# hyllios/CGAT

Measured on AMD Instinct MI355X. Metric: edges/sec through one CGAT attention layer (fwd+bwd), 1M-edge batch, higher is better.
Workload: dtype f32 storage / f16x3c (24-bit operands: exact h + l + t split, 3 fp16 + 3 six-bit matrix passes where built, six bf16 passes elsewhere; fp32 accumulate); 1 GPU; one GATConvNodes layer (H_Net update) fwd+bwd, 4167 crystals x 20 atoms x 12 nbrs per rank: N=83340, E=1000080, C=Ce=128, H=3, scalar attention; edges_per_rank=1000080, parallelism=dp1 (graphs sharded, gradient all-reduce)

## Files before the change

### cgat_amd/_lib.py

```python
import ctypes as C
import os

import torch

_HERE = os.path.dirname(os.path.abspath(__file__))
LIB_PATH = os.path.join(_HERE, "libcgat_hip.so")

MAX_FC = 8
MAX_HYPER = 8
ABI_VERSION = 3

ACT_NONE, ACT_TANH, ACT_LEAKY, ACT_RELU = 0, 1, 2, 3

c_float_p = C.POINTER(C.c_float)
c_i32_p = C.POINTER(C.c_int32)
c_i64_p = C.POINTER(C.c_int64)
vp = C.c_void_p


class Plan(C.Structure):
    _fields_ = [("N", C.c_int32), ("E", C.c_int32), ("dst_rowptr", vp), ("dst_perm", vp), ("dst_sorted", vp),
                ("src_sorted", vp), ("src_rowptr", vp), ("src_pos", vp)]


# ... 106 lines not shown
    "cgat_nodes_attention_bit_form": (C.c_int32, [C.POINTER(Plan), C.POINTER(AttnParams)]),
    "cgat_nodes_attention_infer_workspace_bytes": (C.c_size_t, [C.POINTER(Plan), C.POINTER(AttnParams)]),
    "cgat_nodes_attention_infer": (C.c_int, [C.POINTER(Plan), C.POINTER(AttnParams), vp, vp, vp, vp, C.c_size_t, vp]),
    "cgat_nodes_attention_infer_indexed_ok": (C.c_int32, [C.POINTER(Plan), C.POINTER(AttnParams), C.c_int32]),
    "cgat_nodes_attention_infer_indexed_workspace_bytes": (C.c_size_t, [C.POINTER(Plan), C.POINTER(AttnParams), C.c_int32]),
    "cgat_nodes_attention_infer_indexed": (C.c_int, [C.POINTER(Plan), C.POINTER(AttnParams), vp, vp, C.c_int32, vp, vp, vp,
                                                     C.c_size_t, vp]),
    "cgat_nodes_attention_train_indexed_ok": (C.c_int32, [C.POINTER(Plan), C.POINTER(AttnParams), C.c_int32]),
    "cgat_nodes_attention_indexed_saved_floats": (C.c_size_t, [C.c_int32, C.c_int32, C.c_int32, C.c_int32]),
    "cgat_nodes_attention_forward_indexed_workspace_bytes": (C.c_size_t, [C.POINTER(Plan), C.POINTER(AttnParams), C.c_int32]),
    "cgat_nodes_attention_forward_indexed": (C.c_int, [C.POINTER(Plan), C.POINTER(AttnParams), vp, vp, C.c_int32, vp, vp, vp,
                                                       vp, C.c_size_t, vp]),
    "cgat_nodes_attention_backward_indexed_workspace_bytes": (C.c_size_t, [C.POINTER(Plan), C.POINTER(AttnParams), C.c_int32]),
    "cgat_nodes_attention_backward_indexed": (C.c_int, [C.POINTER(Plan), C.POINTER(AttnParams), vp, vp, C.c_int32, vp, vp, vp,
                                                        vp, vp, vp, vp, vp, C.POINTER(AttnGrads), vp, C.c_size_t, vp]),
    "cgat_indexed_class_pieces": (C.c_int32, [C.c_int32, C.c_int32]),
    "cgat_indexed_class_plan_workspace_bytes": (C.c_size_t, [C.c_int32, C.c_int32]),
    "cgat_indexed_class_plan": (C.c_int, [C.POINTER(Plan), vp, C.c_int32, vp, vp, vp, vp, C.c_size_t, vp]),
    "cgat_debug_nodes_attention_signs_indexed_workspace_bytes": (C.c_size_t, [C.POINTER(Plan), C.POINTER(AttnParams),
                                                                              C.c_int32]),
    "cgat_debug_nodes_attention_signs_indexed": (C.c_int, [C.POINTER(Plan), C.POINTER(AttnParams), vp, vp, C.c_int32, vp, vp,
                                                           vp, C.c_size_t, vp]),
    "cgat_debug_nodes_attention_route": (C.c_uint32, [C.POINTER(Plan), C.POINTER(AttnParams), C.c_int32]),
    "cgat_debug_edge_z_form": (C.c_int, [C.c_int32] * 6 + [C.c_int64] + [C.c_int32] * 5 + [C.POINTER(EdgeZForm)]),
    "cgat_debug_edge_bwd_form": (C.c_int, [C.c_int32] * 11 + [C.POINTER(EdgeBwdForm)]),
    "cgat_debug_nodes_attention_signs": (C.c_int, [C.POINTER(Plan), C.POINTER(AttnParams), vp, vp, vp]),
    "cgat_debug_edge_ge_rebuilt_workspace_bytes": (C.c_size_t, [C.c_int32, C.c_int32, C.c_int32]),
    "cgat_debug_edge_ge_rebuilt": (C.c_int, [vp, vp, vp, vp, vp, vp, vp, C.c_int32, C.c_int32, C.c_int32, vp, vp,
                                             C.c_size_t, vp]),
    "cgat_debug_edge_gw_force_six": (C.c_int32, [C.c_int32]),
    "cgat_debug_edge_gw_rebuilt_workspace_bytes": (C.c_size_t, [C.c_int32, C.c_int32, C.c_int32]),
    "cgat_debug_edge_gw_rebuilt": (C.c_int, [vp, vp, vp, vp, vp, vp, vp, vp, C.c_int32, C.c_int32, C.c_int32, C.c_int32,
                                             vp, C.POINTER(C.c_int32), vp, C.c_size_t, vp]),
    "cgat_hnet_saved_floats": (C.c_size_t, [C.c_int32, C.POINTER(HnetParams)]),
    "cgat_hnet_forward_workspace_bytes": (C.c_size_t, [C.c_int32, C.POINTER(HnetParams)]),
    "cgat_hnet_backward_workspace_bytes": (C.c_size_t, [C.c_int32, C.POINTER(HnetParams)]),
    "cgat_hnet_forward": (C.c_int, [C.c_int32, C.POINTER(HnetParams), vp, vp, vp, vp, vp, C.c_size_t, vp]),
    "cgat_hnet_backward": (C.c_int, [C.c_int32, C.POINTER(HnetParams), vp, vp, vp, vp, vp, vp, C.POINTER(HnetGrads),
                                     vp, C.c_size_t, vp]),
    "cgat_hnet_backward_side_workspace_bytes": (C.c_size_t, [C.c_int32, C.POINTER(HnetParams)]),
    "cgat_hnet_backward_overlapped": (C.c_int, [C.c_int32, C.POINTER(HnetParams), vp, vp, vp, vp, vp, vp,
                                                C.POINTER(HnetGrads), vp, C.c_size_t, vp, vp, C.c_size_t, vp]),
    "cgat_debug_hnet_route": (C.c_uint32, [C.c_int32, C.POINTER(HnetParams), C.c_int32, C.c_int32]),
    "cgat_linear_backward_workspace_bytes": (C.c_size_t, [C.c_int32, C.c_int32, C.c_int32]),
    "cgat_linear_forward_workspace_bytes": (C.c_size_t, [C.c_int32, C.c_int32, C.c_int32]),
    "cgat_linear_forward": (C.c_int, [vp, C.c_int64, vp, C.c_int64, vp, vp, C.c_int64, C.c_int32, C.c_int32,
                                      C.c_int32, C.c_int32, vp, vp, C.c_size_t, vp]),
    "cgat_linear_backward": (C.c_int, [vp, C.c_int64, vp, C.c_int64, vp, C.c_int64, vp, C.c_int64, vp, vp, C.c_int64,
                                       C.c_int32, vp, C.c_int64, vp, C.c_int32, C.c_int32, C.c_int32, C.c_int32, vp,
                                       C.c_size_t, vp]),
    "cgat_segment_softmax_forward": (C.c_int, [vp, vp, vp, C.c_int32, C.c_int32, C.c_float, vp, vp]),
    "cgat_segment_softmax_backward": (C.c_int, [vp, vp, vp, vp, C.c_int32, C.c_int32, vp, vp, vp]),
    "cgat_segment_sum": (C.c_int, [vp, C.c_int64, vp, vp, C.c_int32, C.c_int32, vp, C.c_int64, vp]),
    "cgat_segment_attention_pool_forward": (C.c_int, [vp, C.c_int32, vp, vp, C.c_int64, vp, vp, C.c_int32, C.c_int32, C.c_float,
                                                      vp, vp, vp, vp, vp]),
    "cgat_segment_attention_pool_backward": (C.c_int, [vp, C.c_int32, vp, vp, C.c_int64, vp, vp, C.c_int32, C.c_int32, vp, vp, vp,
                                                       vp, vp, vp, vp, C.c_int64, vp, vp]),
    "cgat_segment_attention_pool_dropout_forward": (C.c_int, [vp, C.c_int32, vp, vp, vp, C.c_int64, vp, vp, C.c_int32,
                                                              C.c_int32, C.c_float, vp, vp, vp, vp, vp]),
    "cgat_segment_attention_pool_dropout_backward": (C.c_int, [vp, C.c_int32, vp, vp, vp, C.c_int64, vp, vp, C.c_int32,
                                                               C.c_int32, vp, vp, vp, vp, vp, vp, vp, C.c_int64, vp]),
    "cgat_edge_head_combine_forward": (C.c_int, [vp, C.c_int32, vp, vp, vp, C.c_int64, C.c_int32, C.c_int32, vp, vp]),
    "cgat_edge_head_combine_backward": (C.c_int, [vp, C.c_int32, vp, vp, vp, vp, C.c_int64, C.c_int32, C.c_int32, vp, vp,
                                                  vp]),
    "cgat_mlp_chain_workspace_bytes": (C.c_size_t, [C.c_int32]),
    "cgat_mlp_chain": (C.c_int, [C.POINTER(ChainDesc), vp, C.c_size_t, vp]),
    "cgat_rowprog_run": (C.c_int, [C.POINTER(RowProg), vp, vp]),
# ... 108 lines not shown
```

### cgat_amd/csrc/edgebwd.hip

```cpp
#include <string.h>
#include "../../include/cgat_hip.h"
#include "common.h"
#include "kernels.h"
#include "mfma_bf16.h"

__device__ __forceinline__ float rc_d(unsigned m, int bit) {
  const unsigned s = (unsigned)((int)(m << (31 - bit)) >> 31);
  return __uint_as_float((s & 0x3F800000u) | (~s & 0x3C23D70Au));
}
__device__ __forceinline__ bf16x8 bits8_bf16(unsigned m) {
  uint4 w;
#define GE_BITPAIR(i_) ((((unsigned)((int)(m << (31 - 2 * (i_))) >> 31)) & 0x3F80u) |                     \
                        (((unsigned)((int)(m << (30 - 2 * (i_))) >> 31)) & 0x3F800000u))
  w.x = GE_BITPAIR(0); w.y = GE_BITPAIR(1); w.z = GE_BITPAIR(2); w.w = GE_BITPAIR(3);
#undef GE_BITPAIR
  return __builtin_bit_cast(bf16x8, w);
}
template <int PASSES, bool RC = false, bool BP = false>
__global__ __launch_bounds__(512, 2) void edge_ge_kernel(const float* __restrict__ gZ, long ldg, long gzb,
                                                         const uint4* __restrict__ Wq, int ncb,
                                                         float* __restrict__ out, long ldo,
                                                         const int* __restrict__ scatter, int E, int accumulate,
                                                         const float* __restrict__ bias,
                                                         const float* __restrict__ amax, const EdgeRC rc, HeadBatch hb) {
// ... 985 lines not shown
}

int edge_gw_launch(const EdgeGwParams& p, hipStream_t stream) {
  if (p.E <= 0) {
    GemmParams z = gemm_params(p.W2, 128, 0, nullptr, 1, nullptr, 1, p.out, p.ldo);
    return gemm_launch(z, nullptr, 0, stream);
  }
  const EdgeGwForm f = edge_gw_form(p);
  CGAT_TRY(edge_gw_check(p, f));
  CGAT_TRY(prepare_T_bf16_rows_launch(p.e, p.lde, p.perm, p.E, p.ws, cdiv(p.E, 128), stream, f.passes == 2 ? p.emax : nullptr));
  if (f.bitplane || f.te_only) {
    {
      CGAT_PROF("edge_gw", stream);
      edge_gw_go(f, p, true, stream);
      CGAT_LAUNCH_CHECK();
    }
    hipLaunchKernelGGL(edge_gw_bit_reduce_kernel, dim3(p.W2 * 4), dim3(256), 0, stream, p.ws + f.slab, f.SM, p.ws + f.slabA, f.SA,
                       p.ws + f.csl, p.rc->wA, p.rc->H, p.rc->HHd, p.W2, f.te_only ? nullptr : p.out, p.ldo, p.te ? *p.te : GwTe{});
    CGAT_LAUNCH_CHECK();
    if (p.te) {
      hipLaunchKernelGGL(gw_te_add_kernel, dim3(cdiv(p.rc->HHd, 256)), dim3(256), 0, stream, p.te->part, p.rc->HHd, p.te->out);
      CGAT_LAUNCH_CHECK();
    }
    if (!f.te_only) return CGAT_OK;
  }
  {
    CGAT_PROF(p.perm ? "edge_gw" : "rows_gw", stream);
    edge_gw_go(f, p, false, stream);
    CGAT_LAUNCH_CHECK();
  }
  return splitk_reduce_launch(p.ws + f.slab, f.S, p.W2, 128, p.out, p.ldo, stream);
}

#define GJ_NODES 4
__global__ __launch_bounds__(256) void edge_gj_kernel(const EdgeRC rc, const int* __restrict__ src_rowptr,
                                                      const int* __restrict__ src_pos, int N, int W2,
                                                      float* __restrict__ Gj, long ldo, float* __restrict__ gjmax) {
  float gmax = 0.f;
  const int per_xcd = gridDim.x / 8;
  const int blk = (blockIdx.x & 7) * per_xcd + (blockIdx.x >> 3);
  const int n0 = blk * GJ_NODES, n1 = min(N, n0 + GJ_NODES);
  for (int q = threadIdx.x; 4 * q < W2; q += 256) {
    const int col = 4 * q;
    const bool isA = col < rc.HHd;
    const int cc = isA ? col : col - rc.HHd, h = cc / rc.Hd;
    const int word = col >> 5, bit = col & 31;
    const float* coef = (isA ? rc.ga : rc.alpha) + h;
    for (int n = n0; n < n1; ++n) {
      const int r0 = src_rowptr[n], r1 = src_rowptr[n + 1];
      float4 acc = make_float4(0.f, 0.f, 0.f, 0.f);
      for (int rb = r0; rb < r1; rb += 4) {
        long t[4];
        float k[4];
        unsigned m[4];
        float4 v[4];
#pragma unroll
        for (int u = 0; u < 4; ++u) t[u] = src_pos[rb + u < r1 ? rb + u : r1 - 1];
#pragma unroll
        for (int u = 0; u < 4; ++u) {
          k[u] = rb + u < r1 ? coef[t[u] * rc.H] : 0.f;
          m[u] = rc.mask[t[u] * rc.nw + word];
          v[u] = *reinterpret_cast<const float4*>(isA ? rc.wA + cc : rc.gS + (long)rc.dst[t[u]] * rc.HHd + cc);
        }
#pragma unroll
        for (int u = 0; u < 4; ++u) {
          const unsigned mb = m[u] >> bit;
          acc.x += (k[u] * v[u].x) * rc_d(mb, 0); acc.y += (k[u] * v[u].y) * rc_d(mb, 1);
          acc.z += (k[u] * v[u].z) * rc_d(mb, 2); acc.w += (k[u] * v[u].w) * rc_d(mb, 3);
        }
      }
      *reinterpret_cast<float4*>(Gj + (long)n * ldo + col) = acc;
      gmax = fmaxf(fmaxf(gmax, fmaxf(fabsf(acc.x), fabsf(acc.y))), fmaxf(fabsf(acc.z), fabsf(acc.w)));
    }
  }
  if (gjmax) block_absmax_commit(gmax, gjmax);
}
int edge_gj_launch(const EdgeRC& rc, const int* src_rowptr, const int* src_pos, int N, int W2, float* Gj, long ldo,
                   hipStream_t stream, float* gjmax) {
  if (N <= 0) return CGAT_OK;
  CGAT_CHECK_ARG(W2 % 4 == 0 && (ldo % 4) == 0 && (((uintptr_t)Gj) & 15) == 0,
                 "edge_gj: W2 = %d must be a multiple of 4 with a 16-byte aligned output", W2);
  CGAT_PROF("edge_gj", stream);
  hipLaunchKernelGGL(edge_gj_kernel, dim3(cdiv(cdiv(N, GJ_NODES), 8) * 8), dim3(256), 0, stream, rc, src_rowptr, src_pos,
                     N, W2, Gj, ldo, gjmax);
  CGAT_LAUNCH_CHECK();
  return CGAT_OK;
}

extern "C" int cgat_debug_edge_bwd_form(int32_t product, int32_t launch, int32_t rows, int32_t W2, int32_t H, int32_t Hd,
                                        int32_t rebuilt, int32_t maxima, int32_t perm, int32_t force_six, int32_t te,
                                        cgat_edge_bwd_form* out) {
  CGAT_CHECK_ARG(out && (product == 0 || product == 1) && launch >= 0 && launch <= (product == 0 ? 3 : 0) && rows >= 0 &&
                 W2 > 0 && W2 % 128 == 0 && H > 0 && Hd > 0, "debug_edge_bwd_form: bad arguments");
  alignas(16) static float present_f;
  static int present_i;
  const EdgeRC rc = edge_rc_shape_only(H, Hd, W2);
  memset(out, 0, sizeof(*out));
  if (product == 1) {
    const EdgeGwParams p = edge_gw_shape(rows, W2, rebuilt ? &rc : nullptr, maxima != 0, perm != 0, force_six != 0, te != 0);
    const EdgeGwForm f = edge_gw_form(p);
    CGAT_TRY(edge_gw_check(p, f));
    out->passes = f.passes; out->rc = f.rc; out->bitplane = f.bitplane; out->grid_x = f.grid_x;
    out->bit_shape = f.bit_shape; out->te_only = f.te_only; out->ranges = f.S; out->SA = f.SA; out->SM = f.SM;
    out->message_pairs = f.npm; out->bit_grid_x = f.bit_grid_x;
    out->ws_end = (int64_t)f.ws_end; out->ws_floats = (int64_t)edge_gw_ws_floats(rows, W2);
    return CGAT_OK;
  }
  EdgeGeParams p = edge_ge_params(&present_f, 128, (long)rows * 128, launch == 2 ? nullptr : &present_f, launch == 3 ? 1 : 128,
                                  launch == 3 ? W2 : 1, &present_f, W2, &present_f, 128, rows);
  if (rebuilt) p.rc = &rc;
  if (maxima) p.amax = &present_f;
  if (perm) p.scatter = &present_i;
  if (launch == 1) { p.slabs = &present_f; p.S = edge_ge_ksplit_groups(rows, W2, rebuilt != 0); }
  if (launch == 3) p.heads = H;
  const EdgeGeForm f = edge_ge_form(p);
  CGAT_TRY(edge_ge_check(p, f));
// ... 5 lines not shown
```

### cgat_amd/csrc/kernels.h

```cpp
#pragma once
#include "common.h"

#define CGAT_ACT_NONE 0
#define CGAT_ACT_TANH 1
#define CGAT_ACT_LEAKY 2
#define CGAT_ACT_RELU 3

struct GemmParams {
  int M, N, K;
  const float* A;
  long lda;
  int a_kmajor;
  const int* a_rgather;
  long a_block;
  const float* B;
  long ldb;
  int b_kmajor;
  const int* b_kgather;
  float* C;
  long ldc;
  const int* c_scatter;
  float alpha, beta;
  const float* bias;
  const float* add1;
// ... 243 lines not shown
struct ChainLayer {
  const uint4* W;
  const float* bias;
  const float* dact;
  const float* resid;
  float* out;
  long ld_dact, ld_resid, ld_out;
  int act;
  int dact_type;
  int accumulate;
};
struct ChainDesc {
  ChainLayer layer[CHAIN_MAX];
  int n_layers, rows;
  const float* x;
  long ldx;
  const float* in_dact;
  long ld_in_dact;
  int in_dact_type;
  float* in_store;
  long ld_in_store;
};
int prepare_W_batch_launch(const WPrepBatch& b, float* dst, hipStream_t stream);
bool mlp_chain128_fast(const ChainDesc& d);
int mlp_chain128_launch(const ChainDesc& d, hipStream_t stream);
#define CHAIN_BATCH_MAX 4
int mlp_chain128_batch_launch(const ChainDesc* d, int n, hipStream_t stream);
int edge_seg_bwd_chunks(int N);
int edge_seg_bwd_launch(const float* Z, float* gZ, long gz_block, const float* alpha, const float* gS, const float* gs,
                        const int* rowptr, const float* wA_out, int N, int H, int Hd, float* tt, float* ga, float* Gi,
                        float* partialW, float* gzmax, unsigned* mask, float* gimax, bool vec, bool zb_6, bool zb,
                        bool rc_shape, bool have_scales, hipStream_t stream,
                        const int* bits_src = nullptr);
int attn_signs_launch(const float* Z, const int* perm, long E, int W2, uint8_t* mask, hipStream_t stream,
                      const unsigned* zbits = nullptr);
struct EdgeRC {
  const unsigned* mask;
  const float* ga;
  const float* alpha;
  const float* gS;
  const float* wA;
  const int* dst;
  int H, Hd, HHd, nw;
  const float* cs;
};
bool edge_mma_bf16();
static inline bool edge_rc_shape(int Ce, int H, int Hd) { return Ce == 128 && H > 0 && Hd > 0 && Hd % 128 == 0; }
struct GwTe {
  const float* We;
  long ldw;
  double* part;
  float* out;
};
struct EdgeGeParams {
  const float* gZ;
  long ldg, gzb;
  const EdgeRC* rc;
  const float* We;
  long s_col, s_out;
  float* Wq;
  int W2;
  int rows;
  float* out;
  long ldo;
  const int* scatter;
  int accumulate;
// ... 49 lines not shown
  const float* gmax;
  const float* emax;
  bool force_six;
  const GwTe* te;
};
static inline EdgeGwParams edge_gw_params(const float* gZ, long ldg, long gzb, const float* e, long lde, const int* perm,
                                          int E, int W2, float* ws, float* out, long ldo) {
  EdgeGwParams p = {};
  p.gZ = gZ; p.ldg = ldg; p.gzb = gzb; p.e = e; p.lde = lde; p.perm = perm; p.E = E; p.W2 = W2; p.ws = ws;
  p.out = out; p.ldo = ldo;
  return p;
}
struct EdgeGwForm {
  int passes;
  bool rc;
  bool bit_shape;
  bool bitplane;
  bool te_only;
  int S, grid_x;
  int SA, SM, npm;
  int bit_grid_x;
  size_t slab;
  size_t slabA, csl;
  size_t ws_end;
};
EdgeGwForm edge_gw_form(const EdgeGwParams& p);
bool edge_gw_bitplane_layer(int H, int Hd);
bool edge_gw_dims(int Ce, int W2, long ldg, long gzb);
size_t edge_gw_ws_floats(int E, int W2);
bool edge_gw_force_six(bool on);
int edge_gw_launch(const EdgeGwParams& p, hipStream_t stream);
int edge_gj_launch(const EdgeRC& rc, const int* src_rowptr, const int* src_pos, int N, int W2, float* Gj, long ldo,
                   hipStream_t stream, float* gjmax = nullptr);

bool rows_dw128_fast(const float* G, long ldg, const float* X1, long ldx1, const float* X2, long ldx2);
size_t rows_dw128_ws_bytes(int rows, int nx);
int rows_dw128_launch(const float* G, long ldg, const float* X1, long ldx1, float* out1, long ldo1, const float* X2,
                      long ldx2, float* out2, long ldo2, float* bsum, int rows, void* ws, size_t ws_bytes,
                      hipStream_t stream);
#define DW_BATCH_MAX 32
struct DwBatchItem {
  const float* G;
  const float* X;
  float* out;
  float* bsum;
};
struct DwBatchDesc {
  int n, rows, splits, rows_per_unit;
  long ldg, ldx, ldo;
  DwBatchItem it[DW_BATCH_MAX];
};
size_t rows_dw128_batch_ws_bytes(int n_items, int rows);
bool rows_dw128_batch_fast(const DwBatchDesc& d);
int rows_dw128_batch_launch(DwBatchDesc d, void* ws, size_t ws_bytes, hipStream_t stream);

int layernorm_tanh_fwd_launch(const float* u, float* y, int rows, int W, float eps, hipStream_t s);
int layernorm_tanh_bwd_launch(const float* u, const float* y, const float* gy, float* gu, int rows, int W, float eps,
                              hipStream_t s);
int act_bwd_launch(const float* y, const float* gy, float* gpre, long n, int act, hipStream_t s);
bool act_bwd_leaky_max_fast(const void* y, const void* gy, const void* gpre, long n);
int act_bwd_leaky_max_launch(const float* y, const float* gy, float* gpre, long n, float* gmax, hipStream_t s);
int colsum_launch(const float* x, long ldx, int rows, int cols, float* out, float alpha, void* ws, size_t ws_bytes,
                  hipStream_t s);
size_t colsum_ws_bytes(int rows, int cols);
int mix_launch(const float* a, const float* b, const float* d, float* out, long n, hipStream_t s);
int mix_bwd_launch(const float* g, const float* a, const float* b, const float* d, float* ga, float* gb_accum,
// ... 49 lines not shown
```

### cgat_amd/csrc/layers.hip

```cpp
#include "layers.h"

struct AttnDims {
  int N, E, C, Ce, H, Hd, D, HHd, W2;
};
static AttnDims attn_dims(const cgat_plan* plan, const cgat_attn_params* p) {
  AttnDims d;
  d.N = plan->N; d.E = plan->E; d.C = p->C; d.Ce = p->Ce; d.H = p->H; d.Hd = p->Hd;
  d.D = 2 * p->C + p->Ce; d.HHd = p->H * p->Hd; d.W2 = 2 * d.HHd;
  return d;
}

struct AttnSaved {
  float *Z, *alpha, *S, *ssum;
};
static AttnSaved attn_saved(float* saved, const AttnDims& d) {
  AttnSaved s;
  s.Z = saved;
  s.alpha = s.Z + (size_t)d.E * d.W2;
  s.S = s.alpha + (size_t)d.E * d.H;
  s.ssum = s.S + (size_t)d.N * d.HHd;
  return s;
}

static int g_edge_storage = -1;
// ... 1369 lines not shown
  EdgeProductDebug q;
  edge_product_debug(q, rc, perm, E);
  q.t.gw_ws = c.take<float>(edge_gw_ws_floats(E, q.d.W2));
  c.seal();
  q.t.e = e; q.t.gWcat = out; q.t.gw_force_six = force_six;
  CGAT_TRY(tail_edge_gw(c, &q.plan, q.d, q.t, tail_route(c.dry, q.d, q.t)));
  return check_ws(c, "debug_edge_gw_rebuilt");
}
extern "C" size_t cgat_debug_edge_gw_rebuilt_workspace_bytes(int32_t E, int32_t H, int32_t Hd) {
  return dry_total([&](Ctx& c) { return debug_edge_gw_impl(c, edge_rc_make(nullptr, nullptr, nullptr, nullptr, nullptr, nullptr, H, Hd), nullptr, nullptr, E, false, nullptr); });
}
extern "C" int cgat_debug_edge_gw_rebuilt(const uint32_t* mask, const float* ga, const float* alpha, const float* gS,
                                          const float* wA, const float* e, const int32_t* perm, const int32_t* dst,
                                          int32_t H, int32_t Hd, int32_t E, int32_t force_six, float* out,
                                          int32_t* took_bitplane, void* ws, size_t ws_bytes, void* stream) {
  const int W2 = 2 * H * Hd;
  CGAT_CHECK_ARG(mask && ga && alpha && gS && wA && e && perm && dst && out && ws, "debug_edge_gw_rebuilt: null pointer");
  if (!mode_split()) {
    cgat_set_error("debug_edge_gw_rebuilt: split arithmetic modes only");
    return CGAT_ERR_UNSUPPORTED;
  }
  CGAT_CHECK_ARG(E > 0 && edge_rc_shape(128, H, Hd) && W2 % 256 == 0, "debug_edge_gw_rebuilt: H = %d, Hd = %d", H, Hd);
  CGAT_CHECK_ARG(ws_bytes >= cgat_debug_edge_gw_rebuilt_workspace_bytes(E, H, Hd) && aligned16(gS, wA, e) && aligned16(out, ws),
                 "debug_edge_gw_rebuilt: workspace too small or operands not 16-byte aligned");
  const EdgeRC rc = edge_rc_make(mask, ga, alpha, gS, wA, dst, H, Hd);
  if (took_bitplane) {
    EdgeGwParams w = edge_gw_params(nullptr, 128, (long)E * 128, e, 128, perm, E, W2, nullptr, out, 128);
    w.rc = &rc; w.force_six = force_six != 0;
    *took_bitplane = edge_gw_form(w).bitplane ? 1 : 0;
  }
  return run_sized("debug_edge_gw_rebuilt", ws, ws_bytes, stream,
                   [&](Ctx& c) { return debug_edge_gw_impl(c, rc, e, perm, E, force_six != 0, out); });
}
```

### cgat_amd/csrc/segbwd.hip

```cpp
#include "common.h"
#include "kernels.h"
#include "mfma_bf16.h"

#define SEGB_NODES 8
#define SEGB_LONG 256
__device__ __forceinline__ float wave_sum_l(float v) {
#pragma unroll
  for (int o = 32; o > 0; o >>= 1) v += __shfl_xor(v, o, 64);
  return v;
}
template <bool VEC, bool ZB = false>
__global__ __launch_bounds__(256) void edge_seg_bwd_kernel(const float* __restrict__ Z, float* __restrict__ gZ,
                                                           long gz_block, const float* __restrict__ alpha,
                                                           const float* __restrict__ gS, const float* __restrict__ gs,
                                                           const int* __restrict__ rowptr,
                                                           const float* __restrict__ wA_out, int N, int H, int Hd,
                                                           float* __restrict__ tt, float* __restrict__ ga,
                                                           float* __restrict__ Gi, float* __restrict__ partialW,
                                                           float* __restrict__ gzmax, unsigned* __restrict__ mask,
                                                           float* __restrict__ gimax) {
  extern __shared__ float pw[];
  float gm = 0.f, gim_max = 0.f;
  const int HHd = H * Hd, W2 = 2 * HHd;
  const int tid = threadIdx.x, lane = tid & 63, wave = tid >> 6;
// ... 363 lines not shown
            w |= (unsigned)__builtin_amdgcn_mov_dpp((int)w, 0x141, 0xF, 0xF, true);
            if ((lane & 7) == 0) mask[(long)t * (W2 >> 5) + (col >> 5)] = w;
            gm = fmaxf(fmaxf(gm, fmaxf(fabsf(g.x), fabsf(g.y))), fmaxf(fabsf(g.z), fabsf(g.w)));
            gi.x += g.x; gi.y += g.y; gi.z += g.z; gi.w += g.w;
          }
        }
      }
      *reinterpret_cast<float4*>(Gi + (long)n * W2 + col) = gi;
      gim_max = fmaxf(fmaxf(gim_max, fmaxf(fabsf(gi.x), fabsf(gi.y))), fmaxf(fabsf(gi.z), fabsf(gi.w)));
      pw[col] += ps.x; pw[col + 1] += ps.y; pw[col + 2] += ps.z; pw[col + 3] += ps.w;
    }
  }
  __syncthreads();
  for (int c = tid; c < HHd; c += 256) partialW[(long)blockIdx.x * HHd + c] = pw[c];
  if (gzmax) block_absmax_commit(gm, gzmax);
  if (gimax) {
    __syncthreads();
    block_absmax_commit(gim_max, gimax);
  }
}

__global__ __launch_bounds__(256, 8) void seg_bwd_attb_kernel(const float* __restrict__ saved, const float* __restrict__ ga,
                                                              const int* __restrict__ rowptr, const int* __restrict__ srcs,
                                                              const float* __restrict__ wA_out, int N, int H,
                                                              float* __restrict__ Gi, float* __restrict__ partialW,
                                                              unsigned* __restrict__ mask) {
  constexpr int Hd = 256;
  extern __shared__ float pw[];
  const int HHd = H * Hd, W2 = 2 * HHd;
  const int tid = threadIdx.x, lane = tid & 63;
  const float* PiA = saved;
  const float* PjA = saved + (long)N * W2;
  const unsigned* zb = reinterpret_cast<const unsigned*>(saved + 2l * N * W2);
  for (int c = tid; c < HHd; c += 256) pw[c] = 0.f;
  __syncthreads();
  const int n0 = blockIdx.x * SEGB_NODES, n1 = min(N, n0 + SEGB_NODES);
  for (int n = n0; n < n1; ++n) {
    const int r0 = __builtin_amdgcn_readfirstlane(rowptr[n]), r1 = __builtin_amdgcn_readfirstlane(rowptr[n + 1]);
    if (r1 == r0) {
      for (int c = tid; c < W2; c += 256) Gi[(long)n * W2 + c] = 0.f;
      continue;
    }
    for (int c4 = tid; c4 < HHd / 4; c4 += 256) {
      const int col = 4 * c4;
      const int h = col / Hd;
      const int bit = col & 31;
      const unsigned* zw = zb + (col >> 5) * 32;
      const unsigned woff = (unsigned)(col >> 5) * 4u;
      const float4 wv = *reinterpret_cast<const float4*>(wA_out + col);
      const float4 pi = *reinterpret_cast<const float4*>(PiA + (long)n * W2 + col);
      float4 gi = make_float4(0.f, 0.f, 0.f, 0.f), ps = gi;
      for (int tb = r0; tb < r1; tb += 4) {
        unsigned m[4];
        float cf[4];
        int sn[4];
        float4 pj[4];
#pragma unroll
        for (int u = 0; u < 4; ++u) {
          const int t = tb + u < r1 ? tb + u : r1 - 1;
          m[u] = zw[(long)(t >> 5) * W2 + (t & 31)];
          cf[u] = ga[(long)t * H + h];
          sn[u] = srcs[t];
        }
#pragma unroll
        for (int u = 0; u < 4; ++u)
          pj[u] = *reinterpret_cast<const float4*>(reinterpret_cast<const char*>(PjA) +
                                                   ((unsigned)sn[u] * (unsigned)W2 + (unsigned)col) * 4u);
#pragma unroll
        for (int u = 0; u < 4; ++u) {
          const int t = tb + u;
          if (t < r1) {
            const unsigned mb = m[u] >> bit;
            const float4 d = make_float4((mb & 1u) ? 1.f : 0.01f, (mb & 2u) ? 1.f : 0.01f, (mb & 4u) ? 1.f : 0.01f,
                                         (mb & 8u) ? 1.f : 0.01f);
            const float gav = cf[u];
            const float4 g = make_float4(gav * wv.x * d.x, gav * wv.y * d.y, gav * wv.z * d.z, gav * wv.w * d.w);
            ps.x += (gav * d.x) * (pi.x + pj[u].x); ps.y += (gav * d.y) * (pi.y + pj[u].y);
            ps.z += (gav * d.z) * (pi.z + pj[u].z); ps.w += (gav * d.w) * (pi.w + pj[u].w);
            if ((lane & 7) == 0) {
              unsigned wo = woff;
              asm volatile("" : "+v"(wo));
              *reinterpret_cast<unsigned*>(reinterpret_cast<char*>(mask + (long)t * (W2 >> 5)) + wo) = m[u];
            }
            gi.x += g.x; gi.y += g.y; gi.z += g.z; gi.w += g.w;
          }
        }
      }
      *reinterpret_cast<float4*>(Gi + (long)n * W2 + col) = gi;
      pw[col] += ps.x; pw[col + 1] += ps.y; pw[col + 2] += ps.z; pw[col + 3] += ps.w;
    }
  }
  __syncthreads();
  for (int c = tid; c < HHd; c += 256) partialW[(long)blockIdx.x * HHd + c] = pw[c];
}

__global__ void attn_signs_kernel(const float* __restrict__ Z, const int* __restrict__ perm, long E, int W2,
                                  uint8_t* __restrict__ mask, const unsigned* __restrict__ zbits) {
  const long i = (long)blockIdx.x * blockDim.x + threadIdx.x;
  if (i >= E * W2) return;
  const long t = i / W2;
  const int c = (int)(i - t * W2);
  if (zbits && c < W2 / 2) mask[(long)perm[t] * W2 + c] = (zbits[(t >> 5) * W2 + (c >> 5) * 32 + (t & 31)] >> (c & 31)) & 1u;
  else mask[(long)perm[t] * W2 + c] = Z[i] > 0.f ? 1 : 0;
}
int attn_signs_launch(const float* Z, const int* perm, long E, int W2, uint8_t* mask, hipStream_t stream,
                      const unsigned* zbits) {
  const long n = E * W2;
  if (n == 0) return CGAT_OK;
  hipLaunchKernelGGL(attn_signs_kernel, dim3((unsigned)cdiv(n, 256)), dim3(256), 0, stream, Z, perm, E, W2, mask, zbits);
  CGAT_LAUNCH_CHECK();
  return CGAT_OK;
}

int edge_seg_bwd_chunks(int N) { return cdiv(N > 0 ? N : 1, SEGB_NODES); }

int seg_bwd_soft_launch(const float* alpha, const float* tt, const int* rowptr, int N, int H, float* ga, hipStream_t stream) {
  CGAT_CHECK_ARG(H >= 1 && H <= 16, "seg_bwd_soft: more than 16 heads");
  if (N <= 0) return CGAT_OK;
  CGAT_PROF("edge_idx_bwd_soft", stream);
  hipLaunchKernelGGL(seg_bwd_soft_kernel, dim3(edge_seg_bwd_chunks(N)), dim3(256), 0, stream, alpha, tt, rowptr, N, H, ga);
  CGAT_LAUNCH_CHECK();
  return CGAT_OK;
}

template <bool ZB>
static int seg_bwd_three_launch(const float* Z, const float* alpha, const float* gS, const float* gs, const int* rowptr,
                                const float* wA_out, int N, int H, float* tt, float* ga, float* Gi, float* partialW,
                                float* gzmax, unsigned* mask, float* gimax, hipStream_t stream,
                                const int* srcs = nullptr) {
  const int chunks = edge_seg_bwd_chunks(N);
  hipLaunchKernelGGL(seg_bwd_msg_kernel<ZB>, dim3((unsigned)cdiv((long)N * H, 4)), dim3(256), 0, stream, Z, alpha, gS, gs, rowptr,
                     N, H, tt, Gi, gzmax, mask, gimax);
  CGAT_LAUNCH_CHECK();
  hipLaunchKernelGGL(seg_bwd_soft_kernel, dim3(chunks), dim3(256), 0, stream, alpha, tt, rowptr, N, H, ga);
  CGAT_LAUNCH_CHECK();
  if (srcs)
    hipLaunchKernelGGL(seg_bwd_attb_kernel, dim3(chunks), dim3(256), (size_t)H * 256 * sizeof(float), stream, Z, ga, rowptr,
                       srcs, wA_out, N, H, Gi, partialW, mask);
  else
  hipLaunchKernelGGL(seg_bwd_att_kernel<ZB>, dim3(chunks), dim3(256), (size_t)H * 256 * sizeof(float), stream, Z, ga, rowptr,
                     wA_out, N, H, Gi, partialW, gzmax, mask, gimax);
  CGAT_LAUNCH_CHECK();
  return CGAT_OK;
}

int edge_seg_bwd_launch(const float* Z, float* gZ, long gz_block, const float* alpha, const float* gS, const float* gs,
                        const int* rowptr, const float* wA_out, int N, int H, int Hd, float* tt, float* ga, float* Gi,
                        float* partialW, float* gzmax, unsigned* mask, float* gimax, bool vec, bool zb_6, bool zb,
                        bool rc_shape, bool have_scales, hipStream_t stream, const int* bits_src) {
  CGAT_CHECK_ARG(H <= 16, "nodes_attention_backward: more than 16 heads");
  CGAT_CHECK_ARG(!bits_src || (vec && mask && Hd == 256 && !zb && !zb_6 && !have_scales),
                 "nodes_attention_backward: the bit form of the saved buffer is the three-kernel fp32 route's");
  CGAT_PROF("edge_seg_bwd", stream);
  if (have_scales) CGAT_TRY(fill_launch(gzmax, 0.f, 8, stream));
  const int chunks = edge_seg_bwd_chunks(N);
  const size_t shm = (size_t)H * Hd * sizeof(float);
  if (zb_6) {
    CGAT_CHECK_ARG(vec && mask && Hd == 256, "nodes_attention_backward: the bf16 edge storage needs the vector form");
    return seg_bwd_three_launch<true>(Z, alpha, gS, gs, rowptr, wA_out, N, H, tt, ga, Gi, partialW, gzmax, mask, gimax, stream);
  }
  if (zb) {
    CGAT_CHECK_ARG(rc_shape && have_scales, "nodes_attention_backward: the bf16 edge storage needs the vector form");
    hipLaunchKernelGGL((edge_seg_bwd_kernel<true, true>), dim3(chunks), dim3(256), shm, stream, Z, gZ, gz_block, alpha, gS,
                       gs, rowptr, wA_out, N, H, Hd, tt, ga, Gi, partialW, gzmax, mask, gimax);
  } else if (vec && mask && Hd == 256) {
    return seg_bwd_three_launch<false>(Z, alpha, gS, gs, rowptr, wA_out, N, H, tt, ga, Gi, partialW, gzmax, mask, gimax, stream,
                                       bits_src);
  } else if (vec)
    hipLaunchKernelGGL(edge_seg_bwd_kernel<true>, dim3(chunks), dim3(256), shm, stream, Z, gZ, gz_block, alpha, gS, gs,
                       rowptr, wA_out, N, H, Hd, tt, ga, Gi, partialW, gzmax, mask, gimax);
  else
// ... 6 lines not shown
```

### cgat_amd/debug.py

```python
import ctypes as C

import torch

from . import _lib
from ._lib import lib, check

last_hidden = None
_active = None


class record_masks:
    def __init__(self, model):
        self.names = {p.data_ptr(): n for n, p in model.named_parameters()}
        self.masks = {}
        self.dropout = []

    def __enter__(self):
        global _active
        self.prev, _active = _active, self
        return self.masks

    def __exit__(self, *exc):
        global _active, last_hidden
        _active = self.prev
# ... 163 lines not shown
    t = [mask.contiguous(), ga.contiguous(), alpha.contiguous(), gS.contiguous(), wA.contiguous(), dst.contiguous(),
         We.contiguous()]
    assert t[0].dtype == torch.int32 and t[5].dtype == torch.int32 and all(v.dtype == torch.float32 for v in t[1:5] + t[6:])
    out = torch.empty(E, 128, dtype=torch.float32, device=dev)
    from . import ops
    nbytes = lib.cgat_debug_edge_ge_rebuilt_workspace_bytes(E, H, Hd)
    ws = ops.workspace(nbytes, dev)
    with torch.cuda.device(dev):
        check(lib.cgat_debug_edge_ge_rebuilt(*[C.c_void_p(v.data_ptr()) for v in t], H, Hd, E, C.c_void_p(out.data_ptr()),
                                             C.c_void_p(ws.data_ptr()), ws.numel() * ws.element_size(),
                                             C.c_void_p(torch.cuda.current_stream().cuda_stream)),
              "cgat_debug_edge_ge_rebuilt")
    return out


def edge_gw_rebuilt(mask, ga, alpha, gS, wA, e, perm, dst, H, Hd, force_six=False):
    E, dev = ga.shape[0], ga.device
    t = [mask.contiguous(), ga.contiguous(), alpha.contiguous(), gS.contiguous(), wA.contiguous(), e.contiguous(),
         perm.contiguous(), dst.contiguous()]
    assert all(v.dtype == torch.int32 for v in (t[0], t[6], t[7])) and all(v.dtype == torch.float32 for v in t[1:6])
    out = torch.empty(2 * H * Hd, 128, dtype=torch.float32, device=dev)
    from . import ops
    ws = ops.workspace(lib.cgat_debug_edge_gw_rebuilt_workspace_bytes(E, H, Hd), dev)
    took = C.c_int32(0)
    with torch.cuda.device(dev):
        check(lib.cgat_debug_edge_gw_rebuilt(*[C.c_void_p(v.data_ptr()) for v in t], H, Hd, E, 1 if force_six else 0,
                                             C.c_void_p(out.data_ptr()), C.byref(took), C.c_void_p(ws.data_ptr()),
                                             ws.numel() * ws.element_size(),
                                             C.c_void_p(torch.cuda.current_stream().cuda_stream)),
              "cgat_debug_edge_gw_rebuilt")
    return out, bool(took.value)


def edge_gw_force_six(flag):
    return bool(lib.cgat_debug_edge_gw_force_six(1 if flag else 0))


def neighbor_tables_with(lattice, frac_coords, atom_ptr, max_neighbor_number, radius, cap, first_radius=0.0):
    from . import neighbors
    return neighbors._run(lattice, frac_coords, atom_ptr, max_neighbor_number, radius, True, True, cap=cap,
                          first_radius=first_radius)
```

### include/cgat_hip.h

```cpp
#ifndef CGAT_HIP_H
#define CGAT_HIP_H
#include <stddef.h>
#include <stdint.h>

#ifdef __cplusplus
extern "C" {
#endif

#define CGAT_ABI_VERSION 3
#define CGAT_MAX_FC 8
#define CGAT_MAX_HYPER 8

int cgat_abi_version(void);
const char* cgat_last_error(void);

void cgat_prof_enable(int on);
void cgat_prof_reset(void);
int cgat_prof_get(const char* tag, int* count, float* total_ms);
uint64_t cgat_prof_launches(void);

typedef struct cgat_plan {
  int32_t N, E;
  const int32_t* dst_rowptr;
  const int32_t* dst_perm;
// ... 177 lines not shown
  int32_t grid_x;
  int32_t groups;
  int32_t blocks_per_group;
  int32_t heads;
  int32_t bit_shape;
  int32_t te_only;
  int32_t ranges;
  int32_t SA, SM;
  int32_t message_pairs;
  int32_t bit_grid_x;
  int32_t reserved;
  int64_t ws_end;
  int64_t ws_floats;
} cgat_edge_bwd_form;
int cgat_debug_edge_bwd_form(int32_t product, int32_t launch, int32_t rows, int32_t W2, int32_t H, int32_t Hd, int32_t rebuilt,
                             int32_t maxima, int32_t perm, int32_t force_six, int32_t te, cgat_edge_bwd_form* out);

int cgat_debug_nodes_attention_signs(const cgat_plan* plan, const cgat_attn_params* p, const float* saved,
                                     uint8_t* mask , void* stream);

int32_t cgat_nodes_attention_bit_form(const cgat_plan* plan, const cgat_attn_params* p);

size_t cgat_debug_edge_ge_rebuilt_workspace_bytes(int32_t E, int32_t H, int32_t Hd);
int cgat_debug_edge_ge_rebuilt(const uint32_t* mask, const float* ga, const float* alpha, const float* gS,
                               const float* wA, const int32_t* dst, const float* We, int32_t H, int32_t Hd, int32_t E,
                               float* out, void* ws, size_t ws_bytes, void* stream);

int32_t cgat_debug_edge_gw_force_six(int32_t on);
size_t cgat_debug_edge_gw_rebuilt_workspace_bytes(int32_t E, int32_t H, int32_t Hd);
int cgat_debug_edge_gw_rebuilt(const uint32_t* mask, const float* ga, const float* alpha, const float* gS,
                               const float* wA, const float* e, const int32_t* perm, const int32_t* dst, int32_t H,
                               int32_t Hd, int32_t E, int32_t force_six, float* out, int32_t* took_bitplane, void* ws,
                               size_t ws_bytes, void* stream);

size_t cgat_edge_hidden_forward_workspace_bytes(const cgat_plan* plan, int32_t C, int32_t Ce, int32_t W2);
size_t cgat_edge_hidden_backward_workspace_bytes(const cgat_plan* plan, int32_t C, int32_t Ce, int32_t W2);
int cgat_edge_hidden_forward(const cgat_plan* plan, int32_t C, int32_t Ce, int32_t W2, const float* w_in ,
                             const float* b_in , const float* x , const float* edge_attr ,
                             float* hidden , float* hidden_absmax ,
                             void* ws, size_t ws_bytes, void* stream);
int cgat_edge_hidden_backward(const cgat_plan* plan, int32_t C, int32_t Ce, int32_t W2, const float* w_in, const float* x,
                              const float* edge_attr, const float* hidden, const float* g_hidden, int32_t g_is_pre,
                              const float* gpre_absmax, float* g_x, float* g_edge_attr, float* g_w_in, float* g_b_in,
                              void* ws, size_t ws_bytes, void* stream);

int32_t cgat_edge_hidden_indexed_ok(const cgat_plan* plan, int32_t C, int32_t Ce, int32_t W2, int32_t R);
size_t cgat_edge_hidden_forward_indexed_workspace_bytes(const cgat_plan* plan, int32_t C, int32_t Ce, int32_t W2, int32_t R);
int cgat_edge_hidden_forward_indexed(const cgat_plan* plan, int32_t C, int32_t Ce, int32_t W2,
                                     const float* w_in , const float* b_in ,
                                     const float* x , const float* table , int32_t R,
                                     const int64_t* index , float* hidden ,
                                     float* hidden_absmax , void* ws, size_t ws_bytes, void* stream);
size_t cgat_edge_hidden_backward_indexed_workspace_bytes(const cgat_plan* plan, int32_t C, int32_t Ce, int32_t W2, int32_t R);
int cgat_edge_hidden_backward_indexed(const cgat_plan* plan, int32_t C, int32_t Ce, int32_t W2, const float* w_in,
                                      const float* x, const float* table, int32_t R, const int64_t* index,
                                      const int32_t* cls_pos, const int32_t* piece_rowptr, const int32_t* piece_start,
                                      const float* hidden, const float* g_hidden, int32_t g_is_pre,
                                      const float* gpre_absmax, float* g_x , float* g_table ,
                                      float* g_w_in , float* g_b_in , void* ws,
                                      size_t ws_bytes, void* stream);

uint32_t cgat_debug_edge_hidden_route(const cgat_plan* plan, int32_t C, int32_t Ce, int32_t W2, int32_t backward,
                                      int32_t g_is_pre, int32_t has_absmax);

typedef struct cgat_hyperlinear_params {
  const float* fc_w[CGAT_MAX_FC];
// ... 219 lines not shown
```

Baseline: 36.10 million edges/s.

## Stage edge indices and coefficients in LDS for edge_gj, XCD-swizzle seg_bwd_attb

Reworks edge_gj so each block covers 8 nodes with up to 1024 threads and stages the edge ids, destinations and per-head ga/alpha coefficients for a contiguous run of edges into shared memory. Threads then sweep the flattened edge range across node boundaries instead of looping node by node. This removes the redundant src_pos/dst/coef global reads made by every column thread and balances work across uneven degrees, at the cost of extra synchronisation and more complex boundary handling with partial-accumulator reloads. seg_bwd_attb gets an XCD-aware block swizzle and its own launcher, and debug entry points are added for both kernels.

```diff
diff --git a/cgat_amd/_lib.py b/cgat_amd/_lib.py
--- a/cgat_amd/_lib.py
+++ b/cgat_amd/_lib.py
@@ -162,7 +162,11 @@
     "cgat_debug_edge_gw_rebuilt_workspace_bytes": (C.c_size_t, [C.c_int32, C.c_int32, C.c_int32]),
     "cgat_debug_edge_gw_rebuilt": (C.c_int, [vp, vp, vp, vp, vp, vp, vp, vp, C.c_int32, C.c_int32, C.c_int32, C.c_int32,
                                              vp, C.POINTER(C.c_int32), vp, C.c_size_t, vp]),
-    "cgat_hnet_saved_floats": (C.c_size_t, [C.c_int32, C.POINTER(HnetParams)]),
+    "cgat_debug_edge_gj_stage_slots": (C.c_int32, []),
+    "cgat_debug_edge_gj": (C.c_int, [vp, vp, vp, vp, vp, vp, vp, vp, C.c_int32, C.c_int32, C.c_int32, vp, vp, vp]),
+    "cgat_debug_seg_bwd_chunks": (C.c_int32, [C.c_int32]),
+    "cgat_debug_seg_bwd_attb": (C.c_int, [vp, vp, vp, vp, vp, C.c_int32, C.c_int32, vp, vp, vp, vp]),
+    "cgat_hnet_saved_floats":(C.c_size_t, [C.c_int32, C.POINTER(HnetParams)]),
     "cgat_hnet_forward_workspace_bytes": (C.c_size_t, [C.c_int32, C.POINTER(HnetParams)]),
     "cgat_hnet_backward_workspace_bytes": (C.c_size_t, [C.c_int32, C.POINTER(HnetParams)]),
     "cgat_hnet_forward": (C.c_int, [C.c_int32, C.POINTER(HnetParams), vp, vp, vp, vp, vp, C.c_size_t, vp]),
diff --git a/cgat_amd/csrc/edgebwd.hip b/cgat_amd/csrc/edgebwd.hip
--- a/cgat_amd/csrc/edgebwd.hip
+++ b/cgat_amd/csrc/edgebwd.hip
@@ -1041,56 +1041,95 @@
   return splitk_reduce_launch(p.ws + f.slab, f.S, p.W2, 128, p.out, p.ldo, stream);
 }
 
-#define GJ_NODES 4
-__global__ __launch_bounds__(256) void edge_gj_kernel(const EdgeRC rc, const int* __restrict__ src_rowptr,
-                                                      const int* __restrict__ src_pos, int N, int W2,
-                                                      float* __restrict__ Gj, long ldo, float* __restrict__ gjmax) {
+#define GJ_NODES 8
+#define GJ_U 4
+__global__ __launch_bounds__(1024) void edge_gj_kernel(const EdgeRC rc, const int* __restrict__ src_rowptr,
+                                                       const int* __restrict__ src_pos, int N, int W2,
+                                                       float* __restrict__ Gj, long ldo, float* __restrict__ gjmax) {
+  extern __shared__ int gj_lds[];
+  __shared__ int rp[GJ_NODES + 1];
+  int* st = gj_lds;
+  int* sd = gj_lds + GJ_STAGE;
+  float* sk = reinterpret_cast<float*>(gj_lds + 2 * GJ_STAGE);
   float gmax = 0.f;
   const int per_xcd = gridDim.x / 8;
   const int blk = (blockIdx.x & 7) * per_xcd + (blockIdx.x >> 3);
-  const int n0 = blk * GJ_NODES, n1 = min(N, n0 + GJ_NODES);
-  for (int q = threadIdx.x; 4 * q < W2; q += 256) {
-    const int col = 4 * q;
-    const bool isA = col < rc.HHd;
-    const int cc = isA ? col : col - rc.HHd, h = cc / rc.Hd;
-    const int word = col >> 5, bit = col & 31;
-    const float* coef = (isA ? rc.ga : rc.alpha) + h;
-    for (int n = n0; n < n1; ++n) {
-      const int r0 = src_rowptr[n], r1 = src_rowptr[n + 1];
-      float4 acc = make_float4(0.f, 0.f, 0.f, 0.f);
-      for (int rb = r0; rb < r1; rb += 4) {
-        long t[4];
-        float k[4];
-        unsigned m[4];
-        float4 v[4];
-#pragma unroll
-        for (int u = 0; u < 4; ++u) t[u] = src_pos[rb + u < r1 ? rb + u : r1 - 1];
-#pragma unroll
-        for (int u = 0; u < 4; ++u) {
-          k[u] = rb + u < r1 ? coef[t[u] * rc.H] : 0.f;
-          m[u] = rc.mask[t[u] * rc.nw + word];
-          v[u] = *reinterpret_cast<const float4*>(isA ? rc.wA + cc : rc.gS + (long)rc.dst[t[u]] * rc.HHd + cc);
+  const int n0 = blk * GJ_NODES, nn = min(N, n0 + GJ_NODES) - n0;
+  const int tid = threadIdx.x, nthr = blockDim.x, nq = W2 >> 2, H = rc.H;
+  if (nn > 0) {
+    if (tid <= nn) rp[tid] = src_rowptr[n0 + tid];
+    __syncthreads();
+    for (int i = 0; i < nn; ++i)
+      if (rp[i + 1] == rp[i])
+        for (int q = tid; q < nq; q += nthr) *reinterpret_cast<float4*>(Gj + (long)(n0 + i) * ldo + 4 * q) = make_float4(0.f, 0.f, 0.f, 0.f);
+    const int R0 = __builtin_amdgcn_readfirstlane(rp[0]), R1 = __builtin_amdgcn_readfirstlane(rp[nn]);
+    for (int p0 = R0; p0 < R1; p0 += GJ_STAGE) {
+      const int cnt = min(R1 - p0, GJ_STAGE);
+      if (p0 != R0) __syncthreads();
+      for (int s = tid; s < cnt; s += nthr) {
+        const long t = src_pos[p0 + s];
+        st[s] = (int)t;
+        sd[s] = rc.dst[t];
+        for (int h = 0; h < H; ++h) { sk[s * 2 * H + h] = rc.ga[t * H + h]; sk[s * 2 * H + H + h] = rc.alpha[t * H + h]; }
+      }
+      __syncthreads();
+      for (int q = tid; q < nq; q += nthr) {
+        const int col = 4 * q;
+        const bool isA = col < rc.HHd;
+        const int cc = isA ? col : col - rc.HHd;
+        const int word = col >> 5, bit = col & 31;
+        const float* coef = sk + (isA ? 0 : H) + cc / rc.Hd;
+        float* orow = Gj + col;
+        int i = -1, r_end = p0;
+        float4 acc = make_float4(0.f, 0.f, 0.f, 0.f);
+        for (int sb = 0; sb < cnt; sb += GJ_U) {
+          float k[GJ_U];
+          unsigned m[GJ_U];
+          float4 v[GJ_U];
+#pragma unroll
+          for (int u = 0; u < GJ_U; ++u) {
+            const int s = sb + u < cnt ? sb + u : cnt - 1;
+            k[u] = coef[s * 2 * H];
+            m[u] = rc.mask[(long)st[s] * rc.nw + word];
+            v[u] = *reinterpret_cast<const float4*>(isA ? rc.wA + cc : rc.gS + (long)sd[s] * rc.HHd + cc);
+          }
+#pragma unroll
+          for (int u = 0; u < GJ_U; ++u) {
+            const int r = p0 + sb + u;
+            if (sb + u < cnt) {
+              if (r >= r_end) {
+                if (i >= 0) {
+                  *reinterpret_cast<float4*>(orow + (long)(n0 + i) * ldo) = acc;
+                  gmax = fmaxf(fmaxf(gmax, fmaxf(fabsf(acc.x), fabsf(acc.y))), fmaxf(fabsf(acc.z), fabsf(acc.w)));
+                }
+                do ++i; while (rp[i + 1] <= r);
+                r_end = __builtin_amdgcn_readfirstlane(rp[i + 1]);
+                acc = rp[i] < p0 ? *reinterpret_cast<const float4*>(orow + (long)(n0 + i) * ldo) : make_float4(0.f, 0.f, 0.f, 0.f);
+              }
+              const unsigned mb = m[u] >> bit;
+              acc.x += (k[u] * v[u].x) * rc_d(mb, 0); acc.y += (k[u] * v[u].y) * rc_d(mb, 1);
+              acc.z += (k[u] * v[u].z) * rc_d(mb, 2); acc.w += (k[u] * v[u].w) * rc_d(mb, 3);
+            }
+          }
         }
-#pragma unroll
-        for (int u = 0; u < 4; ++u) {
-          const unsigned mb = m[u] >> bit;
-          acc.x += (k[u] * v[u].x) * rc_d(mb, 0); acc.y += (k[u] * v[u].y) * rc_d(mb, 1);
-          acc.z += (k[u] * v[u].z) * rc_d(mb, 2); acc.w += (k[u] * v[u].w) * rc_d(mb, 3);
-        }
+        *reinterpret_cast<float4*>(orow + (long)(n0 + i) * ldo) = acc;
+        if (r_end <= p0 + cnt)
+          gmax = fmaxf(fmaxf(gmax, fmaxf(fabsf(acc.x), fabsf(acc.y))), fmaxf(fabsf(acc.z), fabsf(acc.w)));
       }
-      *reinterpret_cast<float4*>(Gj + (long)n * ldo + col) = acc;
-      gmax = fmaxf(fmaxf(gmax, fmaxf(fabsf(acc.x), fabsf(acc.y))), fmaxf(fabsf(acc.z), fabsf(acc.w)));
     }
   }
   if (gjmax) block_absmax_commit(gmax, gjmax);
 }
+static int edge_gj_threads(int W2) { return min(1024, cdiv(W2 / 4, 64) * 64); }
 int edge_gj_launch(const EdgeRC& rc, const int* src_rowptr, const int* src_pos, int N, int W2, float* Gj, long ldo,
                    hipStream_t stream, float* gjmax) {
   if (N <= 0) return CGAT_OK;
   CGAT_CHECK_ARG(W2 % 4 == 0 && (ldo % 4) == 0 && (((uintptr_t)Gj) & 15) == 0,
                  "edge_gj: W2 = %d must be a multiple of 4 with a 16-byte aligned output", W2);
+  CGAT_CHECK_ARG(rc.H >= 1 && rc.H <= 16, "edge_gj: more than 16 heads");
   CGAT_PROF("edge_gj", stream);
-  hipLaunchKernelGGL(edge_gj_kernel, dim3(cdiv(cdiv(N, GJ_NODES), 8) * 8), dim3(256), 0, stream, rc, src_rowptr, src_pos,
+  hipLaunchKernelGGL(edge_gj_kernel, dim3(cdiv(cdiv(N, GJ_NODES), 8) * 8), dim3(edge_gj_threads(W2)),
+                     (size_t)GJ_STAGE * (2 + 2 * rc.H) * sizeof(int), stream, rc, src_rowptr, src_pos,
                      N, W2, Gj, ldo, gjmax);
   CGAT_LAUNCH_CHECK();
   return CGAT_OK;
diff --git a/cgat_amd/csrc/kernels.h b/cgat_amd/csrc/kernels.h
--- a/cgat_amd/csrc/kernels.h
+++ b/cgat_amd/csrc/kernels.h
@@ -299,6 +299,8 @@
                         float* partialW, float* gzmax, unsigned* mask, float* gimax, bool vec, bool zb_6, bool zb,
                         bool rc_shape, bool have_scales, hipStream_t stream,
                         const int* bits_src = nullptr);
+int seg_bwd_attb_launch(const float* saved, const float* ga, const int* rowptr, const int* srcs, const float* wA_out, int N,
+                        int H, float* Gi, float* partialW, unsigned* mask, hipStream_t stream);
 int attn_signs_launch(const float* Z, const int* perm, long E, int W2, uint8_t* mask, hipStream_t stream,
                       const unsigned* zbits = nullptr);
 struct EdgeRC {
@@ -414,6 +416,7 @@
 int edge_gw_launch(const EdgeGwParams& p, hipStream_t stream);
 int edge_gj_launch(const EdgeRC& rc, const int* src_rowptr, const int* src_pos, int N, int W2, float* Gj, long ldo,
                    hipStream_t stream, float* gjmax = nullptr);
+#define GJ_STAGE 256
 
 bool rows_dw128_fast(const float* G, long ldg, const float* X1, long ldx1, const float* X2, long ldx2);
 size_t rows_dw128_ws_bytes(int rows, int nx);
diff --git a/cgat_amd/csrc/layers.hip b/cgat_amd/csrc/layers.hip
--- a/cgat_amd/csrc/layers.hip
+++ b/cgat_amd/csrc/layers.hip
@@ -1425,3 +1425,24 @@
   return run_sized("debug_edge_gw_rebuilt", ws, ws_bytes, stream,
                    [&](Ctx& c) { return debug_edge_gw_impl(c, rc, e, perm, E, force_six != 0, out); });
 }
+
+extern "C" int32_t cgat_debug_edge_gj_stage_slots(void) { return GJ_STAGE; }
+extern "C" int cgat_debug_edge_gj(const uint32_t* mask, const float* ga, const float* alpha, const float* gS, const float* wA,
+                                  const int32_t* dst, const int32_t* rowptr, const int32_t* pos, int32_t N, int32_t H,
+                                  int32_t Hd, float* Gj, float* gjmax, void* stream) {
+  CGAT_CHECK_ARG(mask && ga && alpha && gS && wA && dst && rowptr && pos && Gj, "debug_edge_gj: null pointer");
+  CGAT_CHECK_ARG(N > 0 && H >= 1 && H <= 16 && Hd > 0 && Hd % 32 == 0, "debug_edge_gj: N = %d, H = %d, Hd = %d", N, H, Hd);
+  CGAT_CHECK_ARG(aligned16(gS, wA, Gj), "debug_edge_gj: gS, wA and Gj must be 16-byte aligned");
+  const EdgeRC rc = edge_rc_make(mask, ga, alpha, gS, wA, dst, H, Hd);
+  return edge_gj_launch(rc, rowptr, pos, N, 2 * H * Hd, Gj, 2 * H * Hd, (hipStream_t)stream, gjmax);
+}
+extern "C" int32_t cgat_debug_seg_bwd_chunks(int32_t N) { return edge_seg_bwd_chunks(N); }
+extern "C" int cgat_debug_seg_bwd_attb(const float* saved, const float* ga, const int32_t* rowptr, const int32_t* srcs,
+                                       const float* wA, int32_t N, int32_t H, float* Gi, float* partialW, uint32_t* mask,
+                                       void* stream) {
+  CGAT_CHECK_ARG(saved && ga && rowptr && srcs && wA && Gi && partialW && mask, "debug_seg_bwd_attb: null pointer");
+  CGAT_CHECK_ARG(N > 0 && H >= 1 && H <= 16 && (size_t)N * 2 * H * 256 * 4 < ((size_t)1 << 32),
+                 "debug_seg_bwd_attb: N = %d, H = %d (Hd is 256; N * W2 * 4 bytes below 2^32)", N, H);
+  CGAT_CHECK_ARG(aligned16(saved, wA, Gi), "debug_seg_bwd_attb: saved, wA and Gi must be 16-byte aligned");
+  return seg_bwd_attb_launch(saved, ga, rowptr, srcs, wA, N, H, Gi, partialW, mask, (hipStream_t)stream);
+}
diff --git a/cgat_amd/csrc/segbwd.hip b/cgat_amd/csrc/segbwd.hip
--- a/cgat_amd/csrc/segbwd.hip
+++ b/cgat_amd/csrc/segbwd.hip
@@ -419,9 +419,12 @@
   const float* PiA = saved;
   const float* PjA = saved + (long)N * W2;
   const unsigned* zb = reinterpret_cast<const unsigned*>(saved + 2l * N * W2);
+  const int per_xcd = gridDim.x / 8;
+  const int chunk = (blockIdx.x & 7) * per_xcd + (blockIdx.x >> 3);
+  if (chunk >= (max(N, 1) + SEGB_NODES - 1) / SEGB_NODES) return;
   for (int c = tid; c < HHd; c += 256) pw[c] = 0.f;
   __syncthreads();
-  const int n0 = blockIdx.x * SEGB_NODES, n1 = min(N, n0 + SEGB_NODES);
+  const int n0 = chunk * SEGB_NODES, n1 = min(N, n0 + SEGB_NODES);
   for (int n = n0; n < n1; ++n) {
     const int r0 = __builtin_amdgcn_readfirstlane(rowptr[n]), r1 = __builtin_amdgcn_readfirstlane(rowptr[n + 1]);
     if (r1 == r0) {
@@ -478,7 +481,17 @@
     }
   }
   __syncthreads();
-  for (int c = tid; c < HHd; c += 256) partialW[(long)blockIdx.x * HHd + c] = pw[c];
+  for (int c = tid; c < HHd; c += 256) partialW[(long)chunk * HHd + c] = pw[c];
+}
+
+int seg_bwd_attb_launch(const float* saved, const float* ga, const int* rowptr, const int* srcs, const float* wA_out, int N,
+                        int H, float* Gi, float* partialW, unsigned* mask, hipStream_t stream) {
+  CGAT_CHECK_ARG(H >= 1 && H <= 16, "seg_bwd_attb: more than 16 heads");
+  hipLaunchKernelGGL(seg_bwd_attb_kernel, dim3(cdiv(edge_seg_bwd_chunks(N), 8) * 8), dim3(256),
+                     (size_t)H * 256 * sizeof(float), stream,
+                     saved, ga, rowptr, srcs, wA_out, N, H, Gi, partialW, mask);
+  CGAT_LAUNCH_CHECK();
+  return CGAT_OK;
 }
 
 __global__ void attn_signs_kernel(const float* __restrict__ Z, const int* __restrict__ perm, long E, int W2,
@@ -521,9 +534,7 @@
   CGAT_LAUNCH_CHECK();
   hipLaunchKernelGGL(seg_bwd_soft_kernel, dim3(chunks), dim3(256), 0, stream, alpha, tt, rowptr, N, H, ga);
   CGAT_LAUNCH_CHECK();
-  if (srcs)
-    hipLaunchKernelGGL(seg_bwd_attb_kernel, dim3(chunks), dim3(256), (size_t)H * 256 * sizeof(float), stream, Z, ga, rowptr,
-                       srcs, wA_out, N, H, Gi, partialW, mask);
+  if (srcs) return seg_bwd_attb_launch(Z, ga, rowptr, srcs, wA_out, N, H, Gi, partialW, mask, stream);
   else
   hipLaunchKernelGGL(seg_bwd_att_kernel<ZB>, dim3(chunks), dim3(256), (size_t)H * 256 * sizeof(float), stream, Z, ga, rowptr,
                      wA_out, N, H, Gi, partialW, gzmax, mask, gimax);
diff --git a/cgat_amd/debug.py b/cgat_amd/debug.py
--- a/cgat_amd/debug.py
+++ b/cgat_amd/debug.py
@@ -219,6 +219,42 @@
     return out, bool(took.value)
 
 
+def edge_gj_stage_slots():
+    return int(lib.cgat_debug_edge_gj_stage_slots())
+
+
+def edge_gj(mask, ga, alpha, gS, wA, dst, rowptr, pos, H, Hd, want_max=False):
+    dev = ga.device
+    t = [mask.contiguous(), ga.contiguous(), alpha.contiguous(), gS.contiguous(), wA.contiguous(), dst.contiguous(),
+         rowptr.contiguous(), pos.contiguous()]
+    assert all(v.dtype == torch.int32 for v in (t[0], t[5], t[6], t[7])) and all(v.dtype == torch.float32 for v in t[1:5])
+    N = t[6].numel() - 1
+    out = torch.empty(N, 2 * H * Hd, dtype=torch.float32, device=dev)
+    gmax = torch.zeros(1, dtype=torch.float32, device=dev) if want_max else None
+    with torch.cuda.device(dev):
+        check(lib.cgat_debug_edge_gj(*[C.c_void_p(v.data_ptr()) for v in t], N, H, Hd, C.c_void_p(out.data_ptr()),
+                                     C.c_void_p(gmax.data_ptr()) if want_max else None,
+                                     C.c_void_p(torch.cuda.current_stream().cuda_stream)),
+              "cgat_debug_edge_gj")
+    return (out, gmax) if want_max else out
+
+
+def seg_bwd_attb(saved, ga, rowptr, srcs, wA, N, H):
+    dev = ga.device
+    t = [saved.contiguous(), ga.contiguous(), rowptr.contiguous(), srcs.contiguous(), wA.contiguous()]
+    assert t[2].dtype == torch.int32 and t[3].dtype == torch.int32 and all(v.dtype == torch.float32 for v in (t[0], t[1], t[4]))
+    E, W2 = t[1].shape[0], 2 * H * 256
+    Gi = torch.full((N, W2), float("nan"), dtype=torch.float32, device=dev)
+    pw = torch.empty(int(lib.cgat_debug_seg_bwd_chunks(N)), H * 256, dtype=torch.float32, device=dev)
+    mask = torch.zeros(E, W2 // 32, dtype=torch.int32, device=dev)
+    with torch.cuda.device(dev):
+        check(lib.cgat_debug_seg_bwd_attb(*[C.c_void_p(v.data_ptr()) for v in t], N, H, C.c_void_p(Gi.data_ptr()),
+                                          C.c_void_p(pw.data_ptr()), C.c_void_p(mask.data_ptr()),
+                                          C.c_void_p(torch.cuda.current_stream().cuda_stream)),
+              "cgat_debug_seg_bwd_attb")
+    return Gi, pw, mask
+
+
 def edge_gw_force_six(flag):
     return bool(lib.cgat_debug_edge_gw_force_six(1 if flag else 0))
 
diff --git a/include/cgat_hip.h b/include/cgat_hip.h
--- a/include/cgat_hip.h
+++ b/include/cgat_hip.h
@@ -233,6 +233,16 @@
                                const float* wA, const float* e, const int32_t* perm, const int32_t* dst, int32_t H,
                                int32_t Hd, int32_t E, int32_t force_six, float* out, int32_t* took_bitplane, void* ws,
                                size_t ws_bytes, void* stream);
+
+int32_t cgat_debug_edge_gj_stage_slots(void);
+int cgat_debug_edge_gj(const uint32_t* mask, const float* ga, const float* alpha, const float* gS, const float* wA,
+                       const int32_t* dst, const int32_t* rowptr, const int32_t* pos, int32_t N, int32_t H, int32_t Hd,
+                       float* Gj, float* gjmax, void* stream);
+
+int32_t cgat_debug_seg_bwd_chunks(int32_t N);
+int cgat_debug_seg_bwd_attb(const float* saved, const float* ga, const int32_t* rowptr, const int32_t* srcs,
+                            const float* wA, int32_t N, int32_t H, float* Gi, float* partialW, uint32_t* mask,
+                            void* stream);
 
 size_t cgat_edge_hidden_forward_workspace_bytes(const cgat_plan* plan, int32_t C, int32_t Ce, int32_t W2);
 size_t cgat_edge_hidden_backward_workspace_bytes(const cgat_plan* plan, int32_t C, int32_t Ce, int32_t W2);
```

Measured after the change: 36.16 million edges/s, median of 5. About the same (+0.1%).
